# rogermm14/eonerf_code

Hardware: AMD Instinct MI355X
Metric: train rays/sec on JAX_068 (4096 rays x 128 samples) (higher is better)
Workload: dtype bf16

## Files before the change

eonerf_code_amd/csrc/eonerf_ctx.h:

```cpp
#pragma once
#include <hip/hip_runtime.h>
#include <string.h>
#include <algorithm>
#include <vector>
#include <unordered_map>

#include "../../include/eonerf_hip.h"
#include "eonerf_kernels.h"
#include "eonerf_pack.h"
#include "eonerf_rays.h"
#include "eonerf_carve.h"
#include "eonerf_wgrad_plan.h"

#define HIP_TRY(x) do { hipError_t e_ = (x); if (e_ != hipSuccess) return (int)e_; } while (0)

struct DevStream {
    uint8_t* data = nullptr; size_t bytes = 0;
    ChunkDesc* chunks = nullptr; int n_chunks = 0;
    PackEntry *e16 = nullptr, *e32 = nullptr, *e16lo = nullptr; int n16 = 0, n32 = 0, n16lo = 0;
};

constexpr int RANGE_WORD = 16;
constexpr int RANGE_STICKY_WORD = 17;
constexpr int DIGEST_WORD = 32;

struct eonerf_ctx {
    eonerf_config cfg;
    int n_samples = 128;
    int prec;
    bool bf16;
    int n_cu;
    int enc_pair = 1;
    int pipe_xcd = 0;
    int stagger = 0;
    int wgrad_riders = 1;
    ParamLayout pl;
    DevStream fwd_full, fwd_dens, bwd_full, bwd_dens, bwd_rgb, bwd_full_ig, pipe_wt, bwd_full_heads, bwd_rgb_heads, bwd_dens_heads, ig_tail_wt;
    bool pipe = false;
    int n_pipes = 0;
    float* loss_scratch = nullptr;
    float* fold = nullptr;
    bool pipe_fallback = true;
    bool need_repack = false;
    std::unordered_map<const void*, bool> ws_pipe;
    int pipe_fault_stage = -1;
    bool deterministic = false;
    unsigned long long* pipe_stamps = nullptr;
    uint64_t noise_seed = 0x5eed5eedULL; uint32_t noise_call = 0;
    struct Presample { bool valid = false; const void* ws = nullptr; const float* rays = nullptr; const int64_t* img_idx = nullptr;
                       const float* zsteps = nullptr; const int* count_out = nullptr; int n_rays = 0, flags = 0, n_samples = 0; bool pipe = false; uint32_t call = 0; } pre;
    hipEvent_t exch_event = nullptr; int exch_cus = 0; bool exch_recorded = false;
    const void* pre_consumed_ws = nullptr;
    struct PoseRec { bool valid = false; const void* ws = nullptr; int n_rays = 0, flags = 0, n_samples = 0; bool pipe = false; } pose;
    bool full_ig_dirty = false;
    int* enc_colmap = nullptr;
    int* dev_status = nullptr;
    const uint32_t* occ_bits = nullptr; int occ_r = 0;
    bool weights_set = false;
    bool dens_dirty = false;
    bool dens_used = false;
    int prof_cap = 0;
    std::vector<hipEvent_t> prof_ev[EONERF_PROF_KERNELS][2];
    int prof_n[EONERF_PROF_KERNELS] = {};
};

inline CarveCfg carve_cfg(const eonerf_ctx* ctx) {
    CarveCfg c;
    c.bf16 = ctx->bf16; c.pipe = ctx->pipe; c.deterministic = ctx->deterministic; c.pipe_partials = ctx->deterministic;
    c.n_pipes = ctx->n_pipes; c.n_samples = ctx->n_samples;
    c.enc_part_wgs = (ctx->enc_pair && ctx->pipe && !ctx->deterministic) ? ctx->n_cu : 0;
    return c;
}
inline RenderWs carve_render(const eonerf_ctx* ctx, void* base, int n_rays, int flags) { return carve_render(carve_cfg(ctx), base, n_rays, flags); }

struct ProfScope {
    eonerf_ctx* c; int k; hipStream_t st; bool on;
    ProfScope(eonerf_ctx* ctx, int kernel, hipStream_t s) : c(ctx), k(kernel), st(s), on(kernel >= 0 && ctx->prof_cap > 0 && ctx->prof_n[kernel] < ctx->prof_cap) {
        if (on) (void)hipEventRecord(c->prof_ev[k][0][c->prof_n[k]], st);
    }
    ~ProfScope() { if (on) { (void)hipEventRecord(c->prof_ev[k][1][c->prof_n[k]], st); c->prof_n[k]++; } }
};

inline bool slabs_addressable(const eonerf_ctx* ctx, size_t p_cap) { return slab_blocks_addressable(ctx->bf16, p_cap); }
inline void drop_presample(eonerf_ctx* ctx, const void* ws) { if (ctx->pre.valid && ctx->pre.ws == ws) ctx->pre.valid = false; ctx->pose.valid = false; }
inline bool rays_in_range(const eonerf_ctx* ctx, int n_rays) { return n_rays <= (1 << 24) / (ctx->n_samples > 128 ? ctx->n_samples / 128 : 1); }
inline int chain_grid(const eonerf_ctx* ctx, int p_cap) { return std::min(ctx->n_cu, p_cap / (ctx->bf16 ? PBf16::TILE : PF32::TILE)); }

inline void note_train_forward(eonerf_ctx* ctx, const void* ws) {
    if (ctx->ws_pipe.size() > 1024) ctx->ws_pipe.clear();
    ctx->ws_pipe[ws] = ctx->pipe;
}
struct PipeModeGuard {
    eonerf_ctx* c; bool keep; const void* ws_; bool spend;
    PipeModeGuard(eonerf_ctx* ctx, const void* ws, bool spend_record = true) : c(ctx), keep(ctx->pipe), ws_(ws), spend(spend_record) {
        auto it = c->ws_pipe.find(ws);
        if (it != c->ws_pipe.end()) c->pipe = it->second;
    }
    ~PipeModeGuard() { c->pipe = keep; if (spend) c->ws_pipe.erase(ws_); }
};

inline AmbientW ambient_w(const eonerf_ctx* ctx, const float* flat) {
    const ParamLayout& pl = ctx->pl;
    return AmbientW{flat + pl.t[pl.am1_w].offset, flat + pl.t[pl.am1_b].offset, flat + pl.t[pl.am2_w].offset, flat + pl.t[pl.am2_b].offset};
}

inline int pipe_spare_cus(const eonerf_ctx* ctx) {
    const int spare = ctx->n_cu - ctx->n_pipes * PIPE_STAGES;
    return (ctx->pipe && !ctx->deterministic && spare >= 2) ? std::min(spare, 8) : 0;
}

inline MlpBwdArgs mlp_bwd_args(const eonerf_ctx* ctx, const PassBuffers& b, int p_cap, const DevStream& bs) {
    MlpBwdArgs m;
    memset(&m, 0, sizeof(m));
    m.stagger = ctx->stagger;
    m.n_pts = b.n_pts; m.p_pad = p_cap;
    m.stream = bs.data; m.chunks = bs.chunks; m.n_chunks = bs.n_chunks;
    m.sigma = b.sigma; m.albedo = b.albedo; m.ts = b.ts; m.tb = b.tb;
    m.g_sigma = b.g_sigma; m.g_albedo = b.g_albedo; m.g_ts = b.g_ts; m.g_tb = b.g_tb;
    m.masks = b.masks; m.grd = b.grd; m.g_emb = b.g_emb;
    m.px = b.px; m.py = b.py; m.pz = b.pz; m.g_pos = b.g_pos;
    return m;
}

int eo_pack(const eonerf_ctx* ctx, const std::vector<const DevStream*>& streams, const float* flat, hipStream_t st);
int eo_ensure_density_streams(eonerf_ctx* ctx, const float* flat, hipStream_t st);
int eo_sample_rays(eonerf_ctx* ctx, const float* rays, const float* zsteps, const float* u, int perturb, int n_rays, const uint32_t* bits, int r,
                   int64_t* ray_indices, float* t_starts, float* t_ends, float* pts_per_ray, int* n_dev, void* ws, size_t ws_bytes, void* stream);
int eo_run_mlp_fwd(eonerf_ctx* ctx, const PassBuffers& b, const float* flat, int p_cap, bool full, int mode, hipStream_t st, int prof_id = -1, bool render_train = false);
int eo_run_weight_gradients(eonerf_ctx* ctx, const float* flat, float* d_flat, const PassBuffers* full, const PassBuffers* dens, int p_cap, float* m_bott,
                            int* queue, hipStream_t st, WgradPlanOpts o, float* det_partials = nullptr, BottWgradArgs* defer_bott = nullptr);
```

eonerf_code_amd/csrc/eonerf_ctx.hip:

```cpp
#include <math.h>
#include <new>

#include "eonerf_ctx.h"

namespace {

int upload(DevStream& d, const PackedStream& s) {
    d.bytes = s.bytes; d.n_chunks = (int)s.chunks.size(); d.n16 = (int)s.e16.size(); d.n32 = (int)s.e32.size(); d.n16lo = (int)s.e16lo.size();
    HIP_TRY(hipMalloc(&d.data, s.bytes + 1024));
    HIP_TRY(hipMemset(d.data, 0, s.bytes + 1024));
    HIP_TRY(hipMalloc(&d.chunks, s.chunks.size() * sizeof(ChunkDesc)));
    HIP_TRY(hipMemcpy(d.chunks, s.chunks.data(), s.chunks.size() * sizeof(ChunkDesc), hipMemcpyHostToDevice));
    if (d.n16) {
        HIP_TRY(hipMalloc(&d.e16, s.e16.size() * sizeof(PackEntry)));
        HIP_TRY(hipMemcpy(d.e16, s.e16.data(), s.e16.size() * sizeof(PackEntry), hipMemcpyHostToDevice));
    }
    if (d.n32) {
        HIP_TRY(hipMalloc(&d.e32, s.e32.size() * sizeof(PackEntry)));
        HIP_TRY(hipMemcpy(d.e32, s.e32.data(), s.e32.size() * sizeof(PackEntry), hipMemcpyHostToDevice));
    }
    if (d.n16lo) {
        HIP_TRY(hipMalloc(&d.e16lo, s.e16lo.size() * sizeof(PackEntry)));
        HIP_TRY(hipMemcpy(d.e16lo, s.e16lo.data(), s.e16lo.size() * sizeof(PackEntry), hipMemcpyHostToDevice));
    }
    return 0;
}
void release(DevStream& d) {
    if (d.data) (void)hipFree(d.data);
    if (d.chunks) (void)hipFree(d.chunks);
    if (d.e16) (void)hipFree(d.e16);
    if (d.e32) (void)hipFree(d.e32);
    if (d.e16lo) (void)hipFree(d.e16lo);
    d = DevStream();
}

constexpr int PACK_MAX_JOBS = 16;
struct PackJob { const PackEntry* e; int n; uint8_t* data; int kind; };
struct PackJobs { PackJob j[PACK_MAX_JOBS]; };
__global__ void k_pack(const float* flat, const float* fold, int fold_base, PackJobs jobs, int* range_flag) {
    const PackJob jb = jobs.j[blockIdx.y];
    for (int i = blockIdx.x * blockDim.x + threadIdx.x; i < jb.n; i += gridDim.x * blockDim.x) {
        const PackEntry pe = jb.e[i];
        const float v = pe.src < 0 ? 0.f : (pe.src >= fold_base ? fold[pe.src - fold_base] : flat[pe.src]);
        if (jb.kind == 1) *reinterpret_cast<__bf16*>(jb.data + pe.dst) = (__bf16)v;
        else if (jb.kind == 0) *reinterpret_cast<float*>(jb.data + pe.dst) = v;
        else {
            const _Float16 hi = (_Float16)v;
            *reinterpret_cast<_Float16*>(jb.data + pe.dst) = jb.kind == 2 ? hi : (_Float16)(v - (float)hi);
            if (jb.kind == 2 && !(fabsf(v) <= 65504.f)) atomicOr(range_flag + (RANGE_STICKY_WORD - RANGE_WORD), 1);
        }
    }
}

struct FoldArgs { const float *w_a1, *b_a1, *w_t1, *b_t1, *w_b, *b_b; float* fold; float* wbt; };
__global__ __launch_bounds__(256) void k_fold(FoldArgs a) {
    __shared__ float wat[2][256];
    const int o0 = blockIdx.x * 2, i = threadIdx.x;
#pragma unroll
    for (int r = 0; r < 2; ++r) {
        const int o = o0 + r;
        wat[r][i] = o < 128 ? a.w_a1[(size_t)o * 256 + i] : a.w_t1[(size_t)(o - 128) * 260 + i];
    }
    __syncthreads();
    float acc[2][4] = {{0.f, 0.f, 0.f, 0.f}, {0.f, 0.f, 0.f, 0.f}};
#pragma unroll 16
    for (int k = 0; k < 256; k += 4) {
        float wb[4];
#pragma unroll
        for (int u = 0; u < 4; ++u) wb[u] = a.w_b[(size_t)(k + u) * 256 + i];
#pragma unroll
        for (int u = 0; u < 4; ++u) { acc[0][u] = fmaf(wat[0][k + u], wb[u], acc[0][u]); acc[1][u] = fmaf(wat[1][k + u], wb[u], acc[1][u]); }
    }
#pragma unroll
    for (int r = 0; r < 2; ++r) a.fold[(size_t)(o0 + r) * 256 + i] = (acc[r][0] + acc[r][1]) + (acc[r][2] + acc[r][3]);
#pragma unroll
    for (int r = 0; r < 2; ++r) a.wbt[(size_t)i * 256 + o0 + r] = a.w_b[(size_t)(o0 + r) * 256 + i];
    if (i < 2) {
        const int o = o0 + i;
        float b4[4] = {0.f, 0.f, 0.f, 0.f};
        for (int k = 0; k < 256; ++k) b4[k & 3] = fmaf(wat[i][k], a.b_b[k], b4[k & 3]);
        a.fold[256 * 256 + o] = ((b4[0] + b4[1]) + (b4[2] + b4[3])) + (o < 128 ? a.b_a1[o] : a.b_t1[o - 128]);
    }
}
constexpr float F16X3_W_MAX = 64.f, F16X3_W_MIN = 1.f / 512.f;
struct RangeJob { const float* w; int n; int check_min; };
struct RangeJobs { RangeJob j[24]; };
__global__ __launch_bounds__(256) void k_weight_range(RangeJobs jobs, int* range_flag) {
    __shared__ float red[256];
    __shared__ int bad[1];
    const RangeJob jb = jobs.j[blockIdx.x];
    if (threadIdx.x == 0) bad[0] = 0;
    __syncthreads();
    float m = 0.f;
    for (int i = threadIdx.x; i < jb.n; i += 256) {
        const float v = fabsf(jb.w[i]);
        if (!(v <= 3.0e38f)) bad[0] = 1;
        else m = fmaxf(m, v);
    }
    red[threadIdx.x] = m;
    __syncthreads();
    for (int o = 128; o > 0; o >>= 1) { if ((int)threadIdx.x < o) red[threadIdx.x] = fmaxf(red[threadIdx.x], red[threadIdx.x + o]); __syncthreads(); }
    if (threadIdx.x == 0) {
        const float mx = red[0];
        const float hi_lim = jb.check_min ? F16X3_W_MAX : 65504.f;
        if (bad[0] || mx > hi_lim || (jb.check_min && mx > 0.f && mx < F16X3_W_MIN)) atomicOr(range_flag + (RANGE_STICKY_WORD - RANGE_WORD), 1);
    }
}
int weight_range(const eonerf_ctx* ctx, const float* flat, hipStream_t st) {
    const ParamLayout& pl = ctx->pl;
    RangeJobs jobs;
    int n = 0;
    auto add = [&](int ti, int check_min) { jobs.j[n++] = RangeJob{flat + pl.t[ti].offset, pl.t[ti].rows * pl.t[ti].cols, check_min}; };
    for (int l = 0; l < 8; ++l) add(pl.trunk_w[l], 1);
    add(pl.sig_w, 1); add(pl.a2_w, 1);
    for (int l = 1; l < 4; ++l) add(pl.t_w[l], 1);
    add(pl.tsc_w, 1); add(pl.tbe_w, 1);
    add(pl.t_w[0], 0);
    add(pl.emb, 0);
    jobs.j[n++] = RangeJob{ctx->fold, 256 * 256, 1};
    hipLaunchKernelGGL(k_weight_range, dim3(n), dim3(256), 0, st, jobs, ctx->dev_status + RANGE_WORD);
    return (int)hipGetLastError();
}

int fold_heads(const eonerf_ctx* ctx, const float* flat, hipStream_t st) {
    const ParamLayout& pl = ctx->pl;
    FoldArgs a{flat + pl.t[pl.a1_w].offset, flat + pl.t[pl.a1_b].offset, flat + pl.t[pl.t_w[0]].offset, flat + pl.t[pl.t_b[0]].offset,
               flat + pl.t[pl.bot_w].offset, flat + pl.t[pl.bot_b].offset, ctx->fold, ctx->fold + FOLD_FLOATS};
    hipLaunchKernelGGL(k_fold, dim3(128), dim3(256), 0, st, a);
    return (int)hipGetLastError();
}

constexpr int CLOCK_PROBE_MFMAS = 8192;
typedef __attribute__((ext_vector_type(8))) __bf16 probe_bf16x8;
typedef __attribute__((ext_vector_type(16))) float probe_f32x16;
__global__ __launch_bounds__(256) void k_clock_probe(float* out) {
    probe_bf16x8 a, b;
#pragma unroll
    for (int e = 0; e < 8; ++e) { a[e] = (__bf16)(0.001f * (float)(threadIdx.x + e)); b[e] = (__bf16)(0.002f * (float)(threadIdx.x ^ e)); }
    probe_f32x16 c0 = {}, c1 = {}, c2 = {}, c3 = {};
    const unsigned long long t0 = __builtin_readcyclecounter(), r0 = __builtin_amdgcn_s_memrealtime();
    for (int i = 0; i < CLOCK_PROBE_MFMAS / 4; ++i) {
        c0 = __builtin_amdgcn_mfma_f32_32x32x16_bf16(a, b, c0, 0, 0, 0);
        c1 = __builtin_amdgcn_mfma_f32_32x32x16_bf16(a, b, c1, 0, 0, 0);
        c2 = __builtin_amdgcn_mfma_f32_32x32x16_bf16(a, b, c2, 0, 0, 0);
        c3 = __builtin_amdgcn_mfma_f32_32x32x16_bf16(a, b, c3, 0, 0, 0);
    }
    float s = 0.f;
#pragma unroll
    for (int e = 0; e < 16; ++e) s += (c0[e] + c1[e]) + (c2[e] + c3[e]);
    const unsigned long long t1 = __builtin_readcyclecounter(), r1 = __builtin_amdgcn_s_memrealtime();
    if (blockIdx.x == 0 && threadIdx.x == 0) {
        const float cyc = (float)(t1 - t0), ticks = (float)(r1 - r0);
        out[0] = cyc; out[1] = ticks; out[2] = ticks > 0.f ? cyc / ticks * 100.f : 0.f;
        out[3] = s == 12345.678f ? 1.f : 0.f;
    }
}

}

int eo_pack(const eonerf_ctx* ctx, const std::vector<const DevStream*>& streams, const float* flat, hipStream_t st) {
    PackJobs jobs;
    int n = 0, most = 1;
    auto flush = [&]() {
        if (n) hipLaunchKernelGGL(k_pack, dim3(std::min((most + 255) / 256, 1024), n), dim3(256), 0, st, flat, ctx->fold, (int)ctx->pl.total, jobs, ctx->dev_status + RANGE_WORD);
        n = 0; most = 1;
    };
    for (const DevStream* d : streams) {
        if (n + 3 > PACK_MAX_JOBS) flush();
        if (d->n16) jobs.j[n++] = PackJob{d->e16, d->n16, d->data, d->n16lo ? 2 : 1};
        if (d->n16lo) jobs.j[n++] = PackJob{d->e16lo, d->n16lo, d->data, 3};
        if (d->n32) jobs.j[n++] = PackJob{d->e32, d->n32, d->data, 0};
        most = std::max(most, std::max(d->n16, d->n32));
    }
    flush();
    return (int)hipGetLastError();
}

int eo_ensure_density_streams(eonerf_ctx* ctx, const float* flat, hipStream_t st) {
    ctx->dens_used = true;
    if (!ctx->dens_dirty) return 0;
    const int rc = ctx->prec == EONERF_F16X3 ? eo_pack(ctx, {&ctx->fwd_dens}, flat, st)
                 : ctx->pipe ? eo_pack(ctx, {&ctx->fwd_dens, &ctx->bwd_dens, &ctx->bwd_dens_heads, &ctx->ig_tail_wt}, flat, st)
                             : eo_pack(ctx, {&ctx->fwd_dens, &ctx->bwd_dens}, flat, st);
    if (!rc) ctx->dens_dirty = false;
    return rc;
}

extern "C" {

int eonerf_version(void) { return EONERF_VERSION; }

const char* eonerf_strerror(int code) {
    switch (code) {
        case EONERF_OK: return "ok";
        case EONERF_E_ARG: return "eonerf: invalid argument";
        case EONERF_E_WORKSPACE: return "eonerf: workspace too small";
        case EONERF_E_STATE: return "eonerf: call sequence error (set_weights / train forward missing, or a ray buffer refilled between eonerf_presample and its forward)";
        case EONERF_E_UNSUPPORTED: return "eonerf: unsupported configuration";
        case EONERF_E_RANGE: return "eonerf: a weight, an activation or a position left fp16's range (|v| > 65504 or not finite) in an fp16 x 3 call since the last check; its outputs are invalid -- render in fp32";
        case EONERF_E_DEVICE: return "eonerf: a device-side hand-off timed out (pipelined backward watchdog) on this or another rank; the gradients of that step are invalid and every optimizer update since has been skipped";
        default: return code > 0 ? hipGetErrorString((hipError_t)code) : "eonerf: unknown error";
    }
}

int eonerf_create(eonerf_ctx** out, const eonerf_config* cfg) {
    if (!out || !cfg || cfg->n_images < 1) return EONERF_E_ARG;
    if (cfg->n_samples < 2 || cfg->n_samples > 256) return EONERF_E_UNSUPPORTED;
    if (cfg->precision != EONERF_FP32 && cfg->precision != EONERF_BF16 && cfg->precision != EONERF_F16X3) return EONERF_E_ARG;
    eonerf_ctx* ctx = new (std::nothrow) eonerf_ctx();
    if (!ctx) return EONERF_E_ARG;
    ctx->cfg = *cfg;
    ctx->n_samples = cfg->n_samples;
    ctx->prec = cfg->precision;
    ctx->bf16 = cfg->precision == EONERF_BF16;
    const bool infer_only = cfg->precision == EONERF_F16X3;
    { const char* e = getenv("EONERF_DETERMINISTIC"); ctx->deterministic = e && atoi(e) != 0; }
    int dev = 0;
    hipDeviceProp_t prop;
    if (hipGetDevice(&dev) != hipSuccess || hipGetDeviceProperties(&prop, dev) != hipSuccess) { delete ctx; return (int)hipErrorNoDevice; }
    ctx->n_cu = prop.multiProcessorCount;
    { const char* e = getenv("EONERF_WGRAD_RIDERS"); if (e) ctx->wgrad_riders = atoi(e); }
    { const char* e = getenv("EONERF_STAGGER"); if (e) ctx->stagger = atoi(e); }
    { const char* e = getenv("EONERF_PIPE_XCD"); if (e) ctx->pipe_xcd = atoi(e); }
    { const char* e = getenv("EONERF_ENC_PAIR"); if (e) ctx->enc_pair = atoi(e); }
    ctx->pl.build(cfg->n_images);
    int rc = upload(ctx->fwd_full, build_fwd_stream(ctx->pl, ctx->prec, true));
    if (!rc) rc = upload(ctx->fwd_dens, build_fwd_stream(ctx->pl, ctx->prec, false));
    if (!rc && !infer_only) rc = upload(ctx->bwd_full, build_bwd_stream(ctx->pl, ctx->bf16, true, false));
    if (!rc && !infer_only) rc = upload(ctx->bwd_dens, build_bwd_stream(ctx->pl, ctx->bf16, false, true));
    if (!rc && !infer_only) rc = upload(ctx->bwd_rgb, build_bwd_stream(ctx->pl, ctx->bf16, true, false, false));
    if (!rc && !infer_only) rc = upload(ctx->bwd_full_ig, build_bwd_stream(ctx->pl, ctx->bf16, true, true, true));
    {
        const char* e = getenv("EONERF_PIPE");
        ctx->n_pipes = ctx->n_cu / PIPE_STAGES;
        ctx->pipe = ctx->bf16 && ctx->n_pipes >= 1 && !(e && atoi(e) == 0);
        if (ctx->pipe && !(e && atoi(e) == 1)) {
            if (!eo_bwd_pipe_fits_a_cu() || getenv("HSA_CU_MASK") || getenv("ROC_GLOBAL_CU_MASK")) ctx->pipe = false;
        }
        { const char* fb = getenv("EONERF_PIPE_FALLBACK"); ctx->pipe_fallback = !(fb && atoi(fb) == 0); }
        if (!rc && ctx->pipe) rc = upload(ctx->pipe_wt, build_pipe_stream(ctx->pl));
        if (!rc && ctx->pipe) rc = upload(ctx->bwd_full_heads, build_bwd_stream(ctx->pl, true, true, false, true, 1));
        if (!rc && ctx->pipe) rc = upload(ctx->bwd_rgb_heads, build_bwd_stream(ctx->pl, true, true, false, false, 1));
        if (!rc && ctx->pipe) rc = upload(ctx->bwd_dens_heads, build_bwd_stream(ctx->pl, true, false, true, false, 1));
        if (!rc && ctx->pipe) rc = upload(ctx->ig_tail_wt, build_ig_tail_stream(ctx->pl));
        { const char* f = getenv("EONERF_PIPE_FAULT"); ctx->pipe_fault_stage = f ? atoi(f) : -1; }
        { const char* f = getenv("EONERF_PIPE_STAMPS");
          if (!rc && ctx->pipe && f && atoi(f)) rc = (int)hipMalloc(&ctx->pipe_stamps, (size_t)ctx->n_pipes * PIPE_STAGES * 128 * sizeof(unsigned long long)); }
    }
    if (!rc) rc = (int)hipMalloc(&ctx->fold, (FOLD_FLOATS + 256 * 256) * sizeof(float));
    if (!rc) rc = (int)hipMalloc(&ctx->loss_scratch, (LOSS_MAX_BLOCKS + 4) * sizeof(float));
    if (!rc) rc = (int)hipMemset(ctx->loss_scratch, 0, (LOSS_MAX_BLOCKS + 4) * sizeof(float));
    if (!rc) rc = (int)hipMalloc(&ctx->dev_status, 64 * sizeof(int));
    if (!rc) rc = (int)hipMemset(ctx->dev_status, 0, 64 * sizeof(int));
    if (!rc) {
        int cm[64];
        for (int s = 0; s < 64; ++s) cm[s] = enc_col_of_slot(ctx->bf16, s);
        rc = (int)hipMalloc(&ctx->enc_colmap, sizeof(cm));
        if (!rc) rc = (int)hipMemcpy(ctx->enc_colmap, cm, sizeof(cm), hipMemcpyHostToDevice);
    }
    if (rc) { eonerf_destroy(ctx); return rc; }
    *out = ctx;
    return EONERF_OK;
}

int eonerf_profile_enable(eonerf_ctx* ctx, int max_launches) {
    if (!ctx || max_launches < 0) return EONERF_E_ARG;
    for (int k = 0; k < EONERF_PROF_KERNELS; ++k) {
        for (int s = 0; s < 2; ++s) {
            for (hipEvent_t e : ctx->prof_ev[k][s]) (void)hipEventDestroy(e);
            ctx->prof_ev[k][s].clear();
            for (int i = 0; i < max_launches; ++i) { hipEvent_t e; HIP_TRY(hipEventCreate(&e)); ctx->prof_ev[k][s].push_back(e); }
        }
        ctx->prof_n[k] = 0;
    }
    ctx->prof_cap = max_launches;
    return EONERF_OK;
}

int eonerf_clock_probe(eonerf_ctx* ctx, float* out4, void* stream) {
    if (!ctx || !out4) return EONERF_E_ARG;
    hipLaunchKernelGGL(k_clock_probe, dim3(ctx->n_cu), dim3(256), 0, (hipStream_t)stream, out4);
    return (int)hipGetLastError();
}

const char* eonerf_profile_name(int kernel) {
    static const char* const names[EONERF_PROF_KERNELS] = {"fwd_chain_camera", "bwd_chain_camera", "wgrad_gemm", "fwd_chain_sun", "bwd_chain_sun",
                                                           "bwd_pipe_camera", "bwd_pipe_sun", "ig_tail_sun"};
    return kernel >= 0 && kernel < EONERF_PROF_KERNELS ? names[kernel] : nullptr;
}

int eonerf_profile_read(eonerf_ctx* ctx, int kernel, float* total_ms, int* launches) {
    if (!ctx || kernel < 0 || kernel >= EONERF_PROF_KERNELS || !total_ms || !launches) return EONERF_E_ARG;
    float sum = 0.f;
    for (int i = 0; i < ctx->prof_n[kernel]; ++i) {
        HIP_TRY(hipEventSynchronize(ctx->prof_ev[kernel][1][i]));
        float ms = 0.f;
        HIP_TRY(hipEventElapsedTime(&ms, ctx->prof_ev[kernel][0][i], ctx->prof_ev[kernel][1][i]));
        sum += ms;
    }
    *total_ms = sum; *launches = ctx->prof_n[kernel];
    return EONERF_OK;
}

int eonerf_destroy(eonerf_ctx* ctx) {
    if (!ctx) return EONERF_E_ARG;
    for (int k = 0; k < EONERF_PROF_KERNELS; ++k) for (int s = 0; s < 2; ++s) for (hipEvent_t e : ctx->prof_ev[k][s]) (void)hipEventDestroy(e);
    release(ctx->fwd_full); release(ctx->fwd_dens); release(ctx->bwd_full); release(ctx->bwd_dens); release(ctx->bwd_rgb); release(ctx->bwd_full_ig); release(ctx->pipe_wt); release(ctx->bwd_full_heads); release(ctx->bwd_rgb_heads); release(ctx->bwd_dens_heads); release(ctx->ig_tail_wt);
    if (ctx->fold) (void)hipFree(ctx->fold);
    if (ctx->loss_scratch) (void)hipFree(ctx->loss_scratch);
    if (ctx->enc_colmap) (void)hipFree(ctx->enc_colmap);
    if (ctx->pipe_stamps) (void)hipFree(ctx->pipe_stamps);
    if (ctx->dev_status) (void)hipFree(ctx->dev_status);
    delete ctx;
    return EONERF_OK;
}

int eonerf_param_tensors(const eonerf_ctx* ctx) { return ctx ? (int)ctx->pl.t.size() : 0; }
size_t eonerf_param_floats(const eonerf_ctx* ctx) { return ctx ? ctx->pl.total : 0; }
int eonerf_param_info(const eonerf_ctx* ctx, int index, const char** name, size_t* offset, int* rows, int* cols) {
    if (!ctx || index < 0 || index >= (int)ctx->pl.t.size()) return EONERF_E_ARG;
    const ParamInfo& p = ctx->pl.t[index];
    if (name) *name = p.name.c_str();
    if (offset) *offset = p.offset;
    if (rows) *rows = p.rows;
    if (cols) *cols = p.cols;
    return EONERF_OK;
}

int eonerf_set_weights(eonerf_ctx* ctx, const float* flat, void* stream) {
    if (!ctx || !flat) return EONERF_E_ARG;
    hipStream_t st = (hipStream_t)stream;
    ctx->pose.valid = false;
    std::vector<const DevStream*> v;
    v.push_back(&ctx->fwd_full);
    if (ctx->prec == EONERF_F16X3) {}
    else if (ctx->pipe) { v.push_back(&ctx->bwd_full_heads); v.push_back(&ctx->bwd_rgb_heads); }
    else { v.push_back(&ctx->bwd_full); v.push_back(&ctx->bwd_rgb); }
    if (ctx->pipe) v.push_back(&ctx->pipe_wt);
    const bool with_dens = ctx->dens_used;
    if (with_dens) {
        v.push_back(&ctx->fwd_dens);
        if (ctx->prec != EONERF_F16X3) v.push_back(&ctx->bwd_dens);
        if (ctx->pipe) { v.push_back(&ctx->bwd_dens_heads); v.push_back(&ctx->ig_tail_wt); }
    }
    ctx->need_repack = false;
    int rc = fold_heads(ctx, flat, st);
    if (!rc && ctx->prec == EONERF_F16X3) {
        rc = (int)hipMemsetAsync(ctx->dev_status + RANGE_STICKY_WORD, 0, sizeof(int), st);
        if (!rc) rc = weight_range(ctx, flat, st);
    }
    if (!rc) rc = eo_pack(ctx, v, flat, st);
    if (!rc) { ctx->weights_set = true; ctx->dens_dirty = !with_dens; ctx->full_ig_dirty = true; ctx->dens_used = false; }
    return rc;
}

int eonerf_debug_pipe_stamps(eonerf_ctx* ctx, unsigned long long* host_out, int capacity) {
    if (!ctx || !ctx->pipe_stamps || !host_out) return 0;
    const int n = ctx->n_pipes * PIPE_STAGES * 128;
    if (capacity < n) return 0;
    if (hipDeviceSynchronize() != hipSuccess) return 0;
    if (hipMemcpy(host_out, ctx->pipe_stamps, (size_t)n * sizeof(unsigned long long), hipMemcpyDeviceToHost) != hipSuccess) return 0;
    return n;
}

int eonerf_device_status(eonerf_ctx* ctx, void* stream) {
    if (!ctx) return EONERF_E_ARG;
    int err = 0;
    HIP_TRY(hipMemcpyAsync(&err, ctx->dev_status, sizeof(int), hipMemcpyDeviceToHost, (hipStream_t)stream));
    HIP_TRY(hipStreamSynchronize((hipStream_t)stream));
    if (!err) return EONERF_OK;
    HIP_TRY(hipMemsetAsync(ctx->dev_status, 0, sizeof(int), (hipStream_t)stream));
    if ((err & ~0x100) == EO_STATUS_PRESAMPLE_STALE) return EONERF_E_STATE;
    if (ctx->pipe && ctx->pipe_fallback) { ctx->pipe = false; ctx->need_repack = true; }
    return EONERF_E_DEVICE;
}

int eonerf_range_status(eonerf_ctx* ctx, void* stream) {
    if (!ctx) return EONERF_E_ARG;
    if (ctx->prec != EONERF_F16X3) return EONERF_OK;
    static_assert(RANGE_STICKY_WORD == RANGE_WORD + 1, "both words in one copy");
    int flag[2] = {0, 0};
    HIP_TRY(hipMemcpyAsync(flag, ctx->dev_status + RANGE_WORD, 2 * sizeof(int), hipMemcpyDeviceToHost, (hipStream_t)stream));
    HIP_TRY(hipStreamSynchronize((hipStream_t)stream));
    if (!flag[0] && !flag[1]) return EONERF_OK;
    if (flag[0]) HIP_TRY(hipMemsetAsync(ctx->dev_status + RANGE_WORD, 0, sizeof(int), (hipStream_t)stream));
    return EONERF_E_RANGE;
}

int eonerf_render_status(eonerf_ctx* ctx, int n_rays, int flags, void* ws, size_t ws_bytes, void* stream) {
    (void)n_rays; (void)flags; (void)ws; (void)ws_bytes;
    return eonerf_device_status(ctx, stream);
}

size_t eonerf_grad_floats(const eonerf_ctx* ctx) { return ctx ? ctx->pl.total + 4 : 0; }
size_t eonerf_grad_early_floats(const eonerf_ctx* ctx) { return ctx ? ctx->pl.early : 0; }

int eonerf_set_exchange_event(eonerf_ctx* ctx, void* hip_event, int reserve_cus) {
    if (!ctx || reserve_cus < 0 || reserve_cus > ctx->n_cu / 2) return EONERF_E_ARG;
    ctx->exch_event = (hipEvent_t)hip_event;
    ctx->exch_cus = hip_event ? reserve_cus : 0;
    return EONERF_OK;
}

int eonerf_grad_seal(eonerf_ctx* ctx, float* d_flat, void* stream) {
    if (!ctx || !d_flat) return EONERF_E_ARG;
    return (int)eo_launch_grad_seal(d_flat + ctx->pl.total, ctx->dev_status, (hipStream_t)stream);
}

int eonerf_train_loss(eonerf_ctx* ctx, const float* out, const float* pixels, int n_rays, int kind, float* d_out, float* loss, void* stream) {
    if (!ctx || !out || !pixels || !d_out || !loss || n_rays < 1 || (kind != 0 && kind != 1)) return EONERF_E_ARG;
    return (int)eo_launch_loss(out, pixels, n_rays, kind, d_out, loss, ctx->loss_scratch, (hipStream_t)stream);
}

static int adam_common(eonerf_ctx* ctx, float* flat, float* d_flat, bool zero_grad, float* exp_avg, float* exp_avg_sq,
                       int step, float lr, float beta1, float beta2, float eps, float grad_scale, const float* fault_flag, void* stream) {
    if (!ctx || !flat || !d_flat || !exp_avg || !exp_avg_sq || step < 1) return EONERF_E_ARG;
    hipStream_t st = (hipStream_t)stream;
    HIP_TRY(eo_launch_adam(flat, d_flat, zero_grad, exp_avg, exp_avg_sq, ctx->pl.total, step, lr, beta1, beta2, eps, grad_scale, ctx->dev_status, fault_flag, st));
    return eonerf_set_weights(ctx, flat, stream);
}
int eonerf_adam_step(eonerf_ctx* ctx, float* flat, const float* d_flat, float* exp_avg, float* exp_avg_sq,
                     int step, float lr, float beta1, float beta2, float eps, float grad_scale, const float* fault_flag, void* stream) {
    return adam_common(ctx, flat, const_cast<float*>(d_flat), false, exp_avg, exp_avg_sq, step, lr, beta1, beta2, eps, grad_scale, fault_flag, stream);
}
int eonerf_adam_step_zero_grad(eonerf_ctx* ctx, float* flat, float* d_flat, float* exp_avg, float* exp_avg_sq,
                               int step, float lr, float beta1, float beta2, float eps, float grad_scale, const float* fault_flag, void* stream) {
    return adam_common(ctx, flat, d_flat, true, exp_avg, exp_avg_sq, step, lr, beta1, beta2, eps, grad_scale, fault_flag, stream);
}

}
```

Baseline: 1.251 million.

## Fuse head weight folding into the pack kernel, computing folded entries in place

```diff
diff --git a/eonerf_code_amd/csrc/eonerf_ctx.h b/eonerf_code_amd/csrc/eonerf_ctx.h
--- a/eonerf_code_amd/csrc/eonerf_ctx.h
+++ b/eonerf_code_amd/csrc/eonerf_ctx.h
@@ -18,6 +18,7 @@
     uint8_t* data = nullptr; size_t bytes = 0;
     ChunkDesc* chunks = nullptr; int n_chunks = 0;
     PackEntry *e16 = nullptr, *e32 = nullptr, *e16lo = nullptr; int n16 = 0, n32 = 0, n16lo = 0;
+    PackEntry* ef = nullptr; int nf = 0, kindf = 0;
 };
 
 constexpr int RANGE_WORD = 16;
@@ -40,6 +41,7 @@
     int n_pipes = 0;
     float* loss_scratch = nullptr;
     float* fold = nullptr;
+    bool fold_separate = false;
     bool pipe_fallback = true;
     bool need_repack = false;
     std::unordered_map<const void*, bool> ws_pipe;
@@ -122,7 +124,7 @@
     return m;
 }
 
-int eo_pack(const eonerf_ctx* ctx, const std::vector<const DevStream*>& streams, const float* flat, hipStream_t st);
+int eo_pack(const eonerf_ctx* ctx, const std::vector<const DevStream*>& streams, const float* flat, hipStream_t st, bool heads = false);
 int eo_ensure_density_streams(eonerf_ctx* ctx, const float* flat, hipStream_t st);
 int eo_sample_rays(eonerf_ctx* ctx, const float* rays, const float* zsteps, const float* u, int perturb, int n_rays, const uint32_t* bits, int r,
                    int64_t* ray_indices, float* t_starts, float* t_ends, float* pts_per_ray, int* n_dev, void* ws, size_t ws_bytes, void* stream);
diff --git a/eonerf_code_amd/csrc/eonerf_ctx.hip b/eonerf_code_amd/csrc/eonerf_ctx.hip
--- a/eonerf_code_amd/csrc/eonerf_ctx.hip
+++ b/eonerf_code_amd/csrc/eonerf_ctx.hip
@@ -5,19 +5,47 @@
 
 namespace {
 
-int upload(DevStream& d, const PackedStream& s) {
-    d.bytes = s.bytes; d.n_chunks = (int)s.chunks.size(); d.n16 = (int)s.e16.size(); d.n32 = (int)s.e32.size(); d.n16lo = (int)s.e16lo.size();
+constexpr int FOLD_ROWS = 4;
+
+bool split_fold_entries(std::vector<PackEntry>& list, int fold_base, std::vector<PackEntry>& ef) {
+    auto folded = [&](const PackEntry& e) { return e.src >= fold_base && e.src < fold_base + 256 * 256; };
+    std::vector<PackEntry> f, rest;
+    for (const PackEntry& e : list) (folded(e) ? f : rest).push_back(e);
+    if (f.empty() || f.size() % (FOLD_ROWS * 256)) return false;
+    auto key = [&](const PackEntry& e) { const int k = e.src - fold_base, o = k >> 8, i = k & 255; return ((o / FOLD_ROWS) * 256 + i) * FOLD_ROWS + o % FOLD_ROWS; };
+    std::sort(f.begin(), f.end(), [&](const PackEntry& x, const PackEntry& y) { return key(x) < key(y); });
+    for (size_t n = 0; n < f.size(); ++n) {
+        const int k = f[n].src - fold_base, o = k >> 8, i = k & 255;
+        const int o_first = (f[n - n % (FOLD_ROWS * 256)].src - fold_base) >> 8;
+        if (i != (int)(n / FOLD_ROWS) % 256 || o % FOLD_ROWS != (int)(n % FOLD_ROWS) || o / FOLD_ROWS != o_first / FOLD_ROWS) return false;
+    }
+    list.swap(rest);
+    ef.swap(f);
+    return true;
+}
+
+int upload(DevStream& d, const PackedStream& s, int fold_base = -1) {
+    std::vector<PackEntry> e16 = s.e16, e32 = s.e32, ef;
+    if (fold_base >= 0 && s.e16lo.empty()) {
+        if (split_fold_entries(e16, fold_base, ef)) d.kindf = 1;
+        else if (split_fold_entries(e32, fold_base, ef)) d.kindf = 0;
+    }
+    d.bytes = s.bytes; d.n_chunks = (int)s.chunks.size(); d.n16 = (int)e16.size(); d.n32 = (int)e32.size(); d.n16lo = (int)s.e16lo.size(); d.nf = (int)ef.size();
     HIP_TRY(hipMalloc(&d.data, s.bytes + 1024));
     HIP_TRY(hipMemset(d.data, 0, s.bytes + 1024));
     HIP_TRY(hipMalloc(&d.chunks, s.chunks.size() * sizeof(ChunkDesc)));
     HIP_TRY(hipMemcpy(d.chunks, s.chunks.data(), s.chunks.size() * sizeof(ChunkDesc), hipMemcpyHostToDevice));
     if (d.n16) {
-        HIP_TRY(hipMalloc(&d.e16, s.e16.size() * sizeof(PackEntry)));
-        HIP_TRY(hipMemcpy(d.e16, s.e16.data(), s.e16.size() * sizeof(PackEntry), hipMemcpyHostToDevice));
+        HIP_TRY(hipMalloc(&d.e16, e16.size() * sizeof(PackEntry)));
+        HIP_TRY(hipMemcpy(d.e16, e16.data(), e16.size() * sizeof(PackEntry), hipMemcpyHostToDevice));
     }
     if (d.n32) {
-        HIP_TRY(hipMalloc(&d.e32, s.e32.size() * sizeof(PackEntry)));
-        HIP_TRY(hipMemcpy(d.e32, s.e32.data(), s.e32.size() * sizeof(PackEntry), hipMemcpyHostToDevice));
+        HIP_TRY(hipMalloc(&d.e32, e32.size() * sizeof(PackEntry)));
+        HIP_TRY(hipMemcpy(d.e32, e32.data(), e32.size() * sizeof(PackEntry), hipMemcpyHostToDevice));
+    }
+    if (d.nf) {
+        HIP_TRY(hipMalloc(&d.ef, ef.size() * sizeof(PackEntry)));
+        HIP_TRY(hipMemcpy(d.ef, ef.data(), ef.size() * sizeof(PackEntry), hipMemcpyHostToDevice));
     }
     if (d.n16lo) {
         HIP_TRY(hipMalloc(&d.e16lo, s.e16lo.size() * sizeof(PackEntry)));
@@ -31,17 +59,87 @@
     if (d.e16) (void)hipFree(d.e16);
     if (d.e32) (void)hipFree(d.e32);
     if (d.e16lo) (void)hipFree(d.e16lo);
+    if (d.ef) (void)hipFree(d.ef);
     d = DevStream();
 }
 
-constexpr int PACK_MAX_JOBS = 16;
+constexpr int PACK_MAX_JOBS = 24;
+constexpr int PACK_FOLD = 8, PACK_WBT = 16;
 struct PackJob { const PackEntry* e; int n; uint8_t* data; int kind; };
 struct PackJobs { PackJob j[PACK_MAX_JOBS]; };
-__global__ void k_pack(const float* flat, const float* fold, int fold_base, PackJobs jobs, int* range_flag) {
+struct FoldArgs { const float *w_a1, *b_a1, *w_t1, *b_t1, *w_b, *b_b; float* fold; float* wbt; };
+
+EO_DEV const float* fold_row(const FoldArgs& a, int o) { return o < 128 ? a.w_a1 + (size_t)o * 256 : a.w_t1 + (size_t)(o - 128) * 260; }
+EO_DEV float fold_element(const FoldArgs& a, int k) {
+    const bool bias = k >= 256 * 256;
+    const int o = bias ? k - 256 * 256 : k >> 8;
+    const float* wat = fold_row(a, o);
+    const float* col = bias ? a.b_b : a.w_b + (k & 255);
+    const int ld = bias ? 1 : 256;
+    float acc[4] = {0.f, 0.f, 0.f, 0.f};
+#pragma unroll 1
+    for (int j0 = 0; j0 < 256; j0 += 64) {
+        float w[64], c[64];
+#pragma unroll
+        for (int q = 0; q < 64; ++q) { w[q] = wat[j0 + q]; c[q] = col[(size_t)(j0 + q) * ld]; }
+#pragma unroll
+        for (int q = 0; q < 64; ++q) acc[q & 3] = fmaf(w[q], c[q], acc[q & 3]);
+    }
+    const float s = (acc[0] + acc[1]) + (acc[2] + acc[3]);
+    return bias ? s + (o < 128 ? a.b_a1[o] : a.b_t1[o - 128]) : s;
+}
+EO_DEV void pack_store(uint8_t* data, uint32_t dst, int kind, float v) {
+    if (kind == 1) *reinterpret_cast<__bf16*>(data + dst) = (__bf16)v;
+    else *reinterpret_cast<float*>(data + dst) = v;
+}
+constexpr int FOLD_BLOCK_E = FOLD_ROWS * 64;
+EO_DEV void pack_fold_block(const FoldArgs& a, const PackJob& jb, int fold_base, int vb, float* s_wat, float* s_acc) {
+    const int tid = threadIdx.x, u = tid >> 6, il = tid & 63;
+    const size_t e0 = (size_t)(vb >> 2) * (FOLD_ROWS * 256);
+    const int i = 64 * (vb & 3) + il;
+    float wb[64];
+#pragma unroll
+    for (int q = 0; q < 64; ++q) wb[q] = a.w_b[(size_t)(4 * q + u) * 256 + i];
+    const int o0 = (jb.e[e0].src - fold_base) >> 8;
+    const float* row0 = fold_row(a, o0);
+    const int ld = o0 < 128 ? 256 : 260;
+    float wr[FOLD_ROWS];
+#pragma unroll
+    for (int r = 0; r < FOLD_ROWS; ++r) wr[r] = row0[r * ld + tid];
+#pragma unroll
+    for (int r = 0; r < FOLD_ROWS; ++r) s_wat[r * 256 + tid] = wr[r];
+    __syncthreads();
+    float acc[FOLD_ROWS];
+#pragma unroll
+    for (int r = 0; r < FOLD_ROWS; ++r) acc[r] = 0.f;
+#pragma unroll
+    for (int q = 0; q < 64; ++q)
+#pragma unroll
+        for (int r = 0; r < FOLD_ROWS; ++r) acc[r] = fmaf(s_wat[r * 256 + 4 * q + u], wb[q], acc[r]);
+#pragma unroll
+    for (int r = 0; r < FOLD_ROWS; ++r) s_acc[(u * FOLD_ROWS + r) * 64 + il] = acc[r];
+    __syncthreads();
+    const int r = u;
+    const float v = (s_acc[(0 * FOLD_ROWS + r) * 64 + il] + s_acc[(1 * FOLD_ROWS + r) * 64 + il]) + (s_acc[(2 * FOLD_ROWS + r) * 64 + il] + s_acc[(3 * FOLD_ROWS + r) * 64 + il]);
+    const PackEntry pe = jb.e[e0 + (size_t)i * FOLD_ROWS + r];
+    pack_store(jb.data, pe.dst, jb.kind & 1, v);
+}
+__global__ __launch_bounds__(256) void k_pack(const float* flat, FoldArgs fa, int fold_base, PackJobs jobs, int* range_flag) {
     const PackJob jb = jobs.j[blockIdx.y];
+    if (jb.kind & PACK_FOLD) {
+        __shared__ float s_wat[FOLD_ROWS * 256], s_acc[4 * FOLD_ROWS * 64];
+        static_assert(FOLD_ROWS == 4, "one wave per chain, and wave r finishes row r");
+        for (int vb = blockIdx.x; vb < jb.n / FOLD_BLOCK_E; vb += gridDim.x) pack_fold_block(fa, jb, fold_base, vb, s_wat, s_acc);
+        return;
+    }
+    if (jb.kind == PACK_WBT) {
+        for (int n = blockIdx.x * blockDim.x + threadIdx.x; n < jb.n; n += gridDim.x * blockDim.x)
+            reinterpret_cast<float*>(jb.data)[n] = fa.w_b[(size_t)(n & 255) * 256 + (n >> 8)];
+        return;
+    }
     for (int i = blockIdx.x * blockDim.x + threadIdx.x; i < jb.n; i += gridDim.x * blockDim.x) {
         const PackEntry pe = jb.e[i];
-        const float v = pe.src < 0 ? 0.f : (pe.src >= fold_base ? fold[pe.src - fold_base] : flat[pe.src]);
+        const float v = pe.src < 0 ? 0.f : (pe.src >= fold_base ? (fa.fold ? fa.fold[pe.src - fold_base] : fold_element(fa, pe.src - fold_base)) : flat[pe.src]);
         if (jb.kind == 1) *reinterpret_cast<__bf16*>(jb.data + pe.dst) = (__bf16)v;
         else if (jb.kind == 0) *reinterpret_cast<float*>(jb.data + pe.dst) = v;
         else {
@@ -52,7 +150,6 @@
     }
 }
 
-struct FoldArgs { const float *w_a1, *b_a1, *w_t1, *b_t1, *w_b, *b_b; float* fold; float* wbt; };
 __global__ __launch_bounds__(256) void k_fold(FoldArgs a) {
     __shared__ float wat[2][256];
     const int o0 = blockIdx.x * 2, i = threadIdx.x;
@@ -122,11 +219,13 @@
     return (int)hipGetLastError();
 }
 
+FoldArgs fold_args(const eonerf_ctx* ctx, const float* flat) {
+    const ParamLayout& pl = ctx->pl;
+    return FoldArgs{flat + pl.t[pl.a1_w].offset, flat + pl.t[pl.a1_b].offset, flat + pl.t[pl.t_w[0]].offset, flat + pl.t[pl.t_b[0]].offset,
+                    flat + pl.t[pl.bot_w].offset, flat + pl.t[pl.bot_b].offset, ctx->fold_separate ? ctx->fold : nullptr, ctx->fold + FOLD_FLOATS};
+}
 int fold_heads(const eonerf_ctx* ctx, const float* flat, hipStream_t st) {
-    const ParamLayout& pl = ctx->pl;
-    FoldArgs a{flat + pl.t[pl.a1_w].offset, flat + pl.t[pl.a1_b].offset, flat + pl.t[pl.t_w[0]].offset, flat + pl.t[pl.t_b[0]].offset,
-               flat + pl.t[pl.bot_w].offset, flat + pl.t[pl.bot_b].offset, ctx->fold, ctx->fold + FOLD_FLOATS};
-    hipLaunchKernelGGL(k_fold, dim3(128), dim3(256), 0, st, a);
+    hipLaunchKernelGGL(k_fold, dim3(128), dim3(256), 0, st, fold_args(ctx, flat));
     return (int)hipGetLastError();
 }
 
@@ -158,15 +257,17 @@
 
 }
 
-int eo_pack(const eonerf_ctx* ctx, const std::vector<const DevStream*>& streams, const float* flat, hipStream_t st) {
+int eo_pack(const eonerf_ctx* ctx, const std::vector<const DevStream*>& streams, const float* flat, hipStream_t st, bool heads) {
     PackJobs jobs;
     int n = 0, most = 1;
     auto flush = [&]() {
-        if (n) hipLaunchKernelGGL(k_pack, dim3(std::min((most + 255) / 256, 1024), n), dim3(256), 0, st, flat, ctx->fold, (int)ctx->pl.total, jobs, ctx->dev_status + RANGE_WORD);
+        if (n) hipLaunchKernelGGL(k_pack, dim3(std::min((most + 255) / 256, 1024), n), dim3(256), 0, st, flat, fold_args(ctx, flat), (int)ctx->pl.total, jobs, ctx->dev_status + RANGE_WORD);
         n = 0; most = 1;
     };
+    if (heads && !ctx->fold_separate) { jobs.j[n++] = PackJob{nullptr, 256 * 256, reinterpret_cast<uint8_t*>(ctx->fold + FOLD_FLOATS), PACK_WBT}; most = 256 * 256; }
     for (const DevStream* d : streams) {
-        if (n + 3 > PACK_MAX_JOBS) flush();
+        if (n + 4 > PACK_MAX_JOBS) flush();
+        if (d->nf) jobs.j[n++] = PackJob{d->ef, d->nf, d->data, PACK_FOLD | d->kindf};
         if (d->n16) jobs.j[n++] = PackJob{d->e16, d->n16, d->data, d->n16lo ? 2 : 1};
         if (d->n16lo) jobs.j[n++] = PackJob{d->e16lo, d->n16lo, d->data, 3};
         if (d->n32) jobs.j[n++] = PackJob{d->e32, d->n32, d->data, 0};
@@ -215,6 +316,7 @@
     ctx->bf16 = cfg->precision == EONERF_BF16;
     const bool infer_only = cfg->precision == EONERF_F16X3;
     { const char* e = getenv("EONERF_DETERMINISTIC"); ctx->deterministic = e && atoi(e) != 0; }
+    { const char* e = getenv("EONERF_FOLD_SEPARATE"); ctx->fold_separate = infer_only || (e && atoi(e) != 0); }
     int dev = 0;
     hipDeviceProp_t prop;
     if (hipGetDevice(&dev) != hipSuccess || hipGetDeviceProperties(&prop, dev) != hipSuccess) { delete ctx; return (int)hipErrorNoDevice; }
@@ -224,12 +326,13 @@
     { const char* e = getenv("EONERF_PIPE_XCD"); if (e) ctx->pipe_xcd = atoi(e); }
     { const char* e = getenv("EONERF_ENC_PAIR"); if (e) ctx->enc_pair = atoi(e); }
     ctx->pl.build(cfg->n_images);
-    int rc = upload(ctx->fwd_full, build_fwd_stream(ctx->pl, ctx->prec, true));
-    if (!rc) rc = upload(ctx->fwd_dens, build_fwd_stream(ctx->pl, ctx->prec, false));
-    if (!rc && !infer_only) rc = upload(ctx->bwd_full, build_bwd_stream(ctx->pl, ctx->bf16, true, false));
-    if (!rc && !infer_only) rc = upload(ctx->bwd_dens, build_bwd_stream(ctx->pl, ctx->bf16, false, true));
-    if (!rc && !infer_only) rc = upload(ctx->bwd_rgb, build_bwd_stream(ctx->pl, ctx->bf16, true, false, false));
-    if (!rc && !infer_only) rc = upload(ctx->bwd_full_ig, build_bwd_stream(ctx->pl, ctx->bf16, true, true, true));
+    const int fb = ctx->fold_separate ? -1 : (int)ctx->pl.total;
+    int rc = upload(ctx->fwd_full, build_fwd_stream(ctx->pl, ctx->prec, true), fb);
+    if (!rc) rc = upload(ctx->fwd_dens, build_fwd_stream(ctx->pl, ctx->prec, false), fb);
+    if (!rc && !infer_only) rc = upload(ctx->bwd_full, build_bwd_stream(ctx->pl, ctx->bf16, true, false), fb);
+    if (!rc && !infer_only) rc = upload(ctx->bwd_dens, build_bwd_stream(ctx->pl, ctx->bf16, false, true), fb);
+    if (!rc && !infer_only) rc = upload(ctx->bwd_rgb, build_bwd_stream(ctx->pl, ctx->bf16, true, false, false), fb);
+    if (!rc && !infer_only) rc = upload(ctx->bwd_full_ig, build_bwd_stream(ctx->pl, ctx->bf16, true, true, true), fb);
     {
         const char* e = getenv("EONERF_PIPE");
         ctx->n_pipes = ctx->n_cu / PIPE_STAGES;
@@ -238,11 +341,11 @@
             if (!eo_bwd_pipe_fits_a_cu() || getenv("HSA_CU_MASK") || getenv("ROC_GLOBAL_CU_MASK")) ctx->pipe = false;
         }
         { const char* fb = getenv("EONERF_PIPE_FALLBACK"); ctx->pipe_fallback = !(fb && atoi(fb) == 0); }
-        if (!rc && ctx->pipe) rc = upload(ctx->pipe_wt, build_pipe_stream(ctx->pl));
-        if (!rc && ctx->pipe) rc = upload(ctx->bwd_full_heads, build_bwd_stream(ctx->pl, true, true, false, true, 1));
-        if (!rc && ctx->pipe) rc = upload(ctx->bwd_rgb_heads, build_bwd_stream(ctx->pl, true, true, false, false, 1));
-        if (!rc && ctx->pipe) rc = upload(ctx->bwd_dens_heads, build_bwd_stream(ctx->pl, true, false, true, false, 1));
-        if (!rc && ctx->pipe) rc = upload(ctx->ig_tail_wt, build_ig_tail_stream(ctx->pl));
+        if (!rc && ctx->pipe) rc = upload(ctx->pipe_wt, build_pipe_stream(ctx->pl), fb);
+        if (!rc && ctx->pipe) rc = upload(ctx->bwd_full_heads, build_bwd_stream(ctx->pl, true, true, false, true, 1), fb);
+        if (!rc && ctx->pipe) rc = upload(ctx->bwd_rgb_heads, build_bwd_stream(ctx->pl, true, true, false, false, 1), fb);
+        if (!rc && ctx->pipe) rc = upload(ctx->bwd_dens_heads, build_bwd_stream(ctx->pl, true, false, true, false, 1), fb);
+        if (!rc && ctx->pipe) rc = upload(ctx->ig_tail_wt, build_ig_tail_stream(ctx->pl), fb);
         { const char* f = getenv("EONERF_PIPE_FAULT"); ctx->pipe_fault_stage = f ? atoi(f) : -1; }
         { const char* f = getenv("EONERF_PIPE_STAMPS");
           if (!rc && ctx->pipe && f && atoi(f)) rc = (int)hipMalloc(&ctx->pipe_stamps, (size_t)ctx->n_pipes * PIPE_STAGES * 128 * sizeof(unsigned long long)); }
@@ -344,12 +447,12 @@
         if (ctx->pipe) { v.push_back(&ctx->bwd_dens_heads); v.push_back(&ctx->ig_tail_wt); }
     }
     ctx->need_repack = false;
-    int rc = fold_heads(ctx, flat, st);
+    int rc = ctx->fold_separate ? fold_heads(ctx, flat, st) : 0;
     if (!rc && ctx->prec == EONERF_F16X3) {
         rc = (int)hipMemsetAsync(ctx->dev_status + RANGE_STICKY_WORD, 0, sizeof(int), st);
         if (!rc) rc = weight_range(ctx, flat, st);
     }
-    if (!rc) rc = eo_pack(ctx, v, flat, st);
+    if (!rc) rc = eo_pack(ctx, v, flat, st, true);
     if (!rc) { ctx->weights_set = true; ctx->dens_dirty = !with_dens; ctx->full_ig_dirty = true; ctx->dens_used = false; }
     return rc;
 }
```

Result: no change. 1.251 million, median of 2 (+0.0%).
